# codex-storage/codex-storage-proofs-circuits

Measured on AMD Instinct MI355X. Metric: Poseidon2-BN254 permutations/sec per GPU; full proof-input witnesses/sec, higher is better.
Workload: dtype u32x9 (29-bit limbs, Montgomery mod BN254 r)

## Files before the change

### codex-storage-proofs-circuits_amd/csrc/proof_many.cpp

```cpp
#include <hip/hip_runtime.h>

#include <algorithm>
#include <cstring>
#include <map>
#include <memory>
#include <string>
#include <vector>

#include "dataset_obj.hpp"
#include "proof_input_obj.hpp"
#include "trees.hpp"

using namespace cp2i;

namespace {

struct Req {
  cp2_dataset* ds = nullptr;
  uint64_t slot = 0;
  uint8_t entropy[32];
  size_t at = 0;
  size_t id = 0;
};

// ... 14 lines not shown
    const cp2_dataset* d = ds[i];
    if (!d) return refuse(ctx, i, "NULL dataset");
    if (d->ctx != ctx) return refuse(ctx, i, "its dataset belongs to another context");
    const cp2_config& c = d->cfg;
    if (!same_circuit(c, ds[0]->cfg))
      return refuse(ctx, i, "its circuit parameters (maxDepth, maxLog2NSlots, cellSize, blockSize, nSamples) differ from request 0's");
    const uint64_t s = slot_idx[i];
    if (s < d->first_slot || s - d->first_slot >= d->n_local)
      return refuse(ctx, i, "slot " + std::to_string(s) + " is not local to its dataset (slots " + std::to_string(d->first_slot) + " .. " +
                                std::to_string(d->first_slot + d->n_local - 1) + ")");
    if (!d->have_roots && !(d->first_slot == 0 && d->n_local == c.n_slots))
      return refuse(ctx, i, "its dataset has no dataset tree: not all of its slots are local and cp2_dataset_set_roots was never called");
    const std::string shape = proof_shape_refusal(c, config_slot_tree_depth(c), config_dataset_tree_depth(c));
    if (!shape.empty()) return refuse(ctx, i, shape);
    if (!d->trees && d->tree_mode == 2 && d->csizes.size() - 1 != depth_of(c.n_cells / (c.block_size / c.cell_size)))
      return refuse(ctx, i, "its compact layers do not match its configuration");
  }
  return CP2_OK;
}

int check_roots(cp2_ctx* ctx, cp2_dataset* const* ds, const uint64_t* slot_idx, size_t n) {
  std::vector<uint64_t> a(n);
  for (size_t i = 0; i < n; ++i)
    a[i] = (uint64_t)reinterpret_cast<uintptr_t>(dataset_roots_dev(ds[i])) + (slot_idx[i] - ds[i]->first_slot) * 32;
  std::vector<uint8_t> got(n * 32);
  DevBuf d_a, d_r;
  CP2_TRY(d_a.scratch(ctx, n * 8));
  CP2_TRY(d_r.scratch(ctx, n * 32));
  CP2_HIP(ctx, hipMemcpyAsync(d_a.p, a.data(), n * 8, hipMemcpyHostToDevice, ctx->stream));
  CP2_HIP(ctx, cp2k::launch_gather_addr(static_cast<const uint64_t*>(d_a.p), n, 32, d_r.p, ctx->stream));
  CP2_HIP(ctx, hipMemcpyAsync(got.data(), d_r.p, n * 32, hipMemcpyDeviceToHost, ctx->stream));
  CP2_HIP(ctx, hipStreamSynchronize(ctx->stream));
  for (size_t i = 0; i < n; ++i)
    if (std::memcmp(&got[i * 32], &ds[i]->dlayers[slot_idx[i] * 32], 32) != 0)
      return refuse(ctx, i, "the root its dataset tree holds for slot " + std::to_string(slot_idx[i]) +
                                " (cp2_dataset_set_roots) differs from the slot's built root");
  return CP2_OK;
}

int prepare(cp2_ctx* ctx, cp2_dataset* const* ds, const uint64_t* slot_idx, size_t n) {
  CP2_TRY(validate(ctx, ds, slot_idx, n));
  CP2_HIP(ctx, hipSetDevice(ctx->device));
  std::vector<cp2_dataset*> bare;
  for (size_t i = 0; i < n; ++i)
    if (!ds[i]->have_roots) bare.push_back(ds[i]);
  std::sort(bare.begin(), bare.end());
  bare.erase(std::unique(bare.begin(), bare.end()), bare.end());
  CP2_TRY(set_roots_pass(ctx, bare.data(), nullptr, bare.size(), nullptr));
  return check_roots(ctx, ds, slot_idx, n);
}

std::string who(bool named, const Req* r) { return named ? "request " + std::to_string(r->id) + ": " : std::string(); }

int run_pass(cp2_ctx* ctx, const std::vector<const Req*>& rq, size_t n_rf, size_t n_rfile, size_t n_cf, bool named, cp2_proof_input** out) {
  const size_t n = rq.size(), nr = n_rf + n_rfile;
  const cp2_config& c0 = rq[0]->ds->cfg;
  const size_t ns = c0.n_samples, md = (size_t)c0.max_depth, cs = c0.cell_size, bs = c0.block_size, cpb = bs / cs;
  const size_t T = n * ns, R = nr * ns, C = T - R, RF = n_rf * ns, CF = n_cf * ns;
  auto store = std::make_shared<BatchStore>();
  if (T) {
    std::vector<cp2k::ManyReq> reqs(n);
    std::vector<cp2k::TreeGeom> geoms;
    std::map<std::string, uint32_t> geom_of;
    for (size_t j = 0; j < n; ++j) {
      const cp2_dataset* ds = rq[j]->ds;
      cp2k::ManyReq& q = reqs[j];
      std::memset(&q, 0, sizeof q);
      std::memcpy(q.entropy, rq[j]->entropy, 32);
      std::memcpy(q.slot_root, &ds->dlayers[rq[j]->slot * 32], 32);
      q.n_cells = ds->cfg.n_cells;
      q.cpb = cpb;
      if (j < nr) {
        cp2k::TreeGeom g;
        std::memset(&g, 0, sizeof g);
        trees_geom(ds->trees, &g);
        auto it = geom_of.emplace(std::string(reinterpret_cast<const char*>(&g), sizeof g), (uint32_t)geoms.size());
        if (it.second) geoms.push_back(g);
        q.geom = it.first->second;
        q.nodes = (uint64_t)reinterpret_cast<uintptr_t>(ds->trees->nodes.p);
        q.slot = rq[j]->slot - ds->first_slot;
      }
    }
    std::vector<uint64_t> blk(C), gen, cpaths, ctail, ccell;
    std::vector<uint8_t> checks(2 * C * 32);
    PinBuf h_blocks;
    const size_t rows = T * md + T + 2 * C;
    DevBuf d_req, d_geom, d_idx, d_blk, d_addr, d_rows, d_cells, d_gen, d_caddr;
    CP2_TRY(d_req.scratch(ctx, n * sizeof(cp2k::ManyReq)));
    CP2_TRY(d_geom.scratch(ctx, std::max<size_t>(1, geoms.size()) * sizeof(cp2k::TreeGeom)));
    CP2_TRY(d_idx.scratch(ctx, T * 8));
    CP2_TRY(d_blk.scratch(ctx, T * 8));
    CP2_TRY(d_addr.scratch(ctx, rows * 8));
    CP2_TRY(d_rows.scratch(ctx, rows * 32));
    CP2_TRY(d_cells.scratch(ctx, (C * cpb + T) * cs));
    CP2_TRY(store->idx.alloc(ctx, T * 8));
    CP2_TRY(store->paths.alloc(ctx, T * md * 32));
    CP2_TRY(store->leaves.alloc(ctx, T * 32));
    CP2_TRY(store->cells.alloc(ctx, T * cs));
    uint8_t* cells_out = d_cells.u8() + C * cpb * cs;
    uint64_t* addr = static_cast<uint64_t*>(d_addr.p);
    CP2_HIP(ctx, hipMemcpyAsync(d_req.p, reqs.data(), n * sizeof(cp2k::ManyReq), hipMemcpyHostToDevice, ctx->stream));
    if (!geoms.empty())
      CP2_HIP(ctx, hipMemcpyAsync(d_geom.p, geoms.data(), geoms.size() * sizeof(cp2k::TreeGeom), hipMemcpyHostToDevice, ctx->stream));
    CP2_HIP(ctx, cp2k::launch_sample_many(static_cast<const cp2k::ManyReq*>(d_req.p), static_cast<const cp2k::TreeGeom*>(d_geom.p), n,
                                          (uint32_t)ns, (uint32_t)md, static_cast<uint64_t*>(d_idx.p), static_cast<uint64_t*>(d_blk.p), addr,
                                          ctx->stream));
    CP2_HIP(ctx, hipMemcpyAsync(store->idx.p, d_idx.p, T * 8, hipMemcpyDeviceToHost, ctx->stream));
    if (C) CP2_HIP(ctx, hipMemcpyAsync(blk.data(), static_cast<uint64_t*>(d_blk.p) + R, C * 8, hipMemcpyDeviceToHost, ctx->stream));
    CP2_HIP(ctx, hipStreamSynchronize(ctx->stream));
    const uint64_t* idx = static_cast<const uint64_t*>(store->idx.p);

    gen.assign((CF + RF) * 2, 0);
    uint64_t* seeds = gen.data();
    uint64_t* firsts = seeds + CF + RF;
    for (size_t q = 0; q < CF; ++q) {
      const Req* r = rq[nr + q / ns];
      seeds[q] = cp2_slot_seed(r->ds->cfg.seed, r->slot);
      firsts[q] = blk[q] * cpb;
    }
    for (size_t p = 0; p < RF; ++p) {
      const Req* r = rq[p / ns];
      seeds[CF + p] = cp2_slot_seed(r->ds->cfg.seed, r->slot);
      firsts[CF + p] = idx[p];
    }
    if (CF + RF) {
      CP2_TRY(d_gen.scratch(ctx, gen.size() * 8));
      const uint64_t* dg = static_cast<const uint64_t*>(d_gen.p);
      CP2_HIP(ctx, hipMemcpyAsync(d_gen.p, gen.data(), gen.size() * 8, hipMemcpyHostToDevice, ctx->stream));
      CP2_HIP(ctx, cp2k::launch_gen_fake_cells_many(dg, dg + CF + RF, cpb, CF * cpb, cs, d_cells.p, ctx->stream));
      CP2_HIP(ctx, cp2k::launch_gen_fake_cells_many(dg + CF, dg + CF + RF + CF, 1, RF, cs, cells_out, ctx->stream));
    }
    if (C > CF) {
      const size_t n_req_file = (C - CF) / ns;
      CP2_TRY(h_blocks.alloc(ctx, (C - CF) * bs));
      std::vector<std::string> failed(fill_threads(ctx));
      on_threads(fill_threads(ctx), n_req_file, [&](int w, size_t k) {
        const size_t q0 = CF + k * ns;
        const Req* r = rq[nr + q0 / ns];
        const std::string fname = slot_file_name(r->ds->file_base, r->slot);
        size_t bad = 0;
        const int err = slot_file_read_list(fname, ns, [&](size_t) { return bs; }, [&](size_t c) { return blk[q0 + c] * bs; },
                                            [&](size_t c) { return h_blocks.u8() + (q0 - CF + c) * bs; }, &bad);
        if (err >= 0)
          failed[w] = who(named, r) + (err ? "block " + std::to_string(blk[q0 + bad]) + " of slot " : std::string("slot ")) + std::to_string(r->slot) +
                      ": " + slot_file_error(fname, err);
        return err < 0;
      });
      for (const auto& f : failed)
        if (!f.empty()) { ctx->err = f; return CP2_ERR_IO; }
      CP2_HIP(ctx, hipMemcpyAsync(d_cells.u8() + CF * bs, h_blocks.p, (C - CF) * bs, hipMemcpyHostToDevice, ctx->stream));
    }
    cp2_slot_trees* mini = nullptr;
    struct Mini { cp2_slot_trees*& t; ~Mini() { cp2_slot_trees_free(t); } } mini_guard{mini};
    if (C) {
      cpaths.assign(C * md, 0);
      ctail.assign(3 * C, 0);
      ccell.assign(C, 0);
      CP2_TRY(cp2_slot_trees_build_dev(ctx, d_cells.p, C, cs, bs, cpb, &mini));
      const size_t depth_b = depth_of(cpb);
      const uint64_t mb = (uint64_t)reinterpret_cast<uintptr_t>(mini->nodes.p);
      std::vector<uint64_t> rr(depth_b + 1);
      for (size_t q = 0; q < C; ++q) {
        const Req* r = rq[nr + q / ns];
        const cp2_dataset* ds = r->ds;
        const uint64_t ls = r->slot - ds->first_slot, cell = idx[R + q], b = blk[q], in_block = cell % cpb;
        const uint64_t kb = (uint64_t)reinterpret_cast<uintptr_t>(ds->compact.p);
        uint64_t* P = &cpaths[q * md];
        path_rows(mini, q, in_block, depth_b + 1, rr.data());
        for (size_t d = 0; d < depth_b; ++d) P[d] = rr[d] == NO_ROW ? 0 : mb + rr[d] * 32;
        uint64_t j = b, m = ds->cfg.n_cells / cpb;
        for (size_t d = 0; d + 1 < ds->csizes.size(); ++d) {
          const uint64_t sib = j ^ 1;
          P[depth_b + d] = sib < m ? kb + (ds->coff[d] + ls * ds->csizes[d] + sib) * 32 : 0;
          j >>= 1;
          m = (m + 1) >> 1;
        }
        ctail[q] = mb + (q * cpb + in_block) * 32;
        ctail[C + 2 * q] = kb + (ds->coff[0] + ls * ds->csizes[0] + b) * 32;
        ctail[C + 2 * q + 1] = mb + (mini->toff[0] + q) * 32;
        ccell[q] = (uint64_t)reinterpret_cast<uintptr_t>(d_cells.u8()) + (q * cpb + in_block) * cs;
      }
      CP2_TRY(d_caddr.scratch(ctx, C * 8));
      CP2_HIP(ctx, hipMemcpyAsync(addr + R * md, cpaths.data(), C * md * 8, hipMemcpyHostToDevice, ctx->stream));
      CP2_HIP(ctx, hipMemcpyAsync(addr + T * md + R, ctail.data(), 3 * C * 8, hipMemcpyHostToDevice, ctx->stream));
      CP2_HIP(ctx, hipMemcpyAsync(d_caddr.p, ccell.data(), C * 8, hipMemcpyHostToDevice, ctx->stream));
      CP2_HIP(ctx, cp2k::launch_gather_addr(static_cast<const uint64_t*>(d_caddr.p), C, cs, cells_out + R * cs, ctx->stream));
    }
    CP2_HIP(ctx, cp2k::launch_gather_addr(addr, rows, 32, d_rows.p, ctx->stream));
    CP2_HIP(ctx, hipMemcpyAsync(store->paths.p, d_rows.p, T * md * 32, hipMemcpyDeviceToHost, ctx->stream));
    CP2_HIP(ctx, hipMemcpyAsync(store->leaves.p, d_rows.u8() + T * md * 32, T * 32, hipMemcpyDeviceToHost, ctx->stream));
    if (C) CP2_HIP(ctx, hipMemcpyAsync(checks.data(), d_rows.u8() + (T * md + T) * 32, 2 * C * 32, hipMemcpyDeviceToHost, ctx->stream));
    CP2_HIP(ctx, hipMemcpyAsync(store->cells.p, cells_out, T * cs, hipMemcpyDeviceToHost, ctx->stream));
    CP2_HIP(ctx, hipStreamSynchronize(ctx->stream));
    for (size_t q = 0; q < C; ++q)
      if (std::memcmp(&checks[2 * q * 32], &checks[(2 * q + 1) * 32], 32) != 0) {
        const Req* r = rq[nr + q / ns];
        ctx->err = who(named, r) + "block " + std::to_string(blk[q]) + " of slot " + std::to_string(r->slot) +
                   " does not hash to its stored root (slot data changed since the build?)";
        return CP2_ERR_IO;
      }
    if (R > RF) {
      std::vector<std::string> failed(fill_threads(ctx));
      on_threads(fill_threads(ctx), n_rfile, [&](int w, size_t k) {
        const Req* r = rq[n_rf + k];
        const std::string fname = slot_file_name(r->ds->file_base, r->slot);
        const size_t p0 = (n_rf + k) * ns;
        const int err = slot_file_read_list(fname, ns, [&](size_t) { return cs; }, [&](size_t c) { return idx[p0 + c] * cs; },
                                            [&](size_t c) { return store->cells.u8() + (p0 + c) * cs; });
        if (err >= 0) failed[w] = who(named, r) + slot_file_error(fname, err);
        return err < 0;
      });
      for (const auto& f : failed)
        if (!f.empty()) { ctx->err = f; return CP2_ERR_IO; }
    }
  }
  std::vector<ProofItem> items(n);
  for (size_t j = 0; j < n; ++j) items[j] = {rq[j]->ds, rq[j]->slot, rq[j]->entropy, &out[rq[j]->at]};
  return proof_inputs_from_store(items.data(), n, store, store->cells.u8());
}

}

int cp2i::prove_requests(cp2_ctx* ctx, cp2_dataset* const* ds, const uint64_t* slot_idx, const uint8_t* entropies, size_t n, size_t at0,
                         bool named, cp2_proof_input** out) {
  for (size_t i = 0; i < n; ++i) out[i] = nullptr;
  if (n == 0) return CP2_OK;
  CP2_HIP(ctx, hipSetDevice(ctx->device));
  std::vector<Req> req(n);
  std::vector<const Req*> res_fake, res_file, cmp_fake, cmp_file, roots_only;
  for (size_t i = 0; i < n; ++i) {
    req[i].ds = ds[i];
    req[i].slot = slot_idx[i];
    req[i].at = i;
    req[i].id = at0 + i;
    canonical_felt(entropies + 32 * i, req[i].entropy);
    const cp2_dataset* d = ds[i];
    (d->trees ? (d->from_file ? res_file : res_fake) : d->tree_mode == 2 ? (d->from_file ? cmp_file : cmp_fake) : roots_only).push_back(&req[i]);
  }
  auto fail = [&](int st) {
    for (size_t i = 0; i < n; ++i) { cp2_proof_input_free(out[i]); out[i] = nullptr; }
    return st;
  };
  for (const Req* r : roots_only) {
    const int st = cp2_proof_inputs_generate_batch(r->ds, &r->slot, 1, r->entropy, &out[r->at]);
    if (st != CP2_OK) {
      ctx->err = who(named, r) + ctx->err;
      return fail(st);
    }
  }
  const cp2_config& c0 = ds[0]->cfg;
  const size_t per_req = std::max<size_t>(1, (size_t)c0.n_samples * c0.block_size);
  const size_t chunk = std::max<size_t>(1, ctx->stage_bytes / per_req);
  std::vector<const Req*> compact(cmp_fake);
  compact.insert(compact.end(), cmp_file.begin(), cmp_file.end());
  const size_t n_res = res_fake.size() + res_file.size();
  size_t c = 0;
  for (bool first = true; first ? n_res + compact.size() > 0 : c < compact.size(); first = false) {
    std::vector<const Req*> rq;
    if (first) {
      rq = res_fake;
      rq.insert(rq.end(), res_file.begin(), res_file.end());
    }
    const size_t c1 = std::min(compact.size(), c + chunk);
    rq.insert(rq.end(), compact.begin() + (long)c, compact.begin() + (long)c1);
    const size_t n_cf = c < cmp_fake.size() ? std::min(c1, cmp_fake.size()) - c : 0;
    const int st = run_pass(ctx, rq, first ? res_fake.size() : 0, first ? res_file.size() : 0, n_cf, named, out);
    if (st != CP2_OK) return fail(st);
    c = c1;
  }
  return CP2_OK;
}

extern "C" int cp2_proof_inputs_generate_many(cp2_ctx* ctx, cp2_dataset* const* ds, const uint64_t* slot_idx, const uint8_t* entropies, size_t n,
                                              cp2_proof_input** out) try {
  if (!ctx) return CP2_ERR_INVALID;
  if (n && (!ds || !slot_idx || !entropies || !out)) {
    ctx->err = "cp2_proof_inputs_generate_many: NULL array";
    return CP2_ERR_INVALID;
  }
  for (size_t i = 0; i < n; ++i) out[i] = nullptr;
  if (n == 0) return CP2_OK;
  CP2_REFUSE_STUCK(ctx);
  CP2_TRY(prepare(ctx, ds, slot_idx, n));
  return prove_requests(ctx, ds, slot_idx, entropies, n, 0, true, out);
} catch (const std::bad_alloc&) {
  return CP2_ERR_ALLOC;
} catch (...) {
  return CP2_ERR_INVALID;
}

extern "C" int cp2_proof_inputs_export_many(cp2_ctx* ctx, cp2_dataset* const* ds, const uint64_t* slot_idx, const uint8_t* entropies, size_t n,
                                            const char* const* paths, int threads, size_t batch, uint64_t* total_bytes) try {
  if (!ctx) return CP2_ERR_INVALID;
  if (n && (!ds || !slot_idx || !entropies)) {
    ctx->err = "cp2_proof_inputs_export_many: NULL array";
    return CP2_ERR_INVALID;
  }
  if (total_bytes) *total_bytes = 0;
  if (n == 0) return CP2_OK;
  CP2_REFUSE_STUCK(ctx);
  CP2_TRY(prepare(ctx, ds, slot_idx, n));
  return export_in_chunks(n, batch, threads, [&](size_t b0, size_t m, cp2_proof_input** out) {
    return prove_requests(ctx, ds + b0, slot_idx + b0, entropies + 32 * b0, m, b0, true, out);
  }, [&](size_t i) { return paths ? paths[i] : nullptr; }, total_bytes);
} catch (const std::bad_alloc&) {
  return CP2_ERR_ALLOC;
} catch (...) {
  return CP2_ERR_INVALID;
}
```

### codex-storage-proofs-circuits_amd/csrc/slot_trees.cpp

```cpp
#include <hip/hip_runtime.h>

#include <fcntl.h>
#include <sys/mman.h>
#include <sys/stat.h>
#include <unistd.h>

#include <algorithm>
#include <atomic>
#include <chrono>
#include <cstdio>
#include <cstdlib>
#include <cstring>
#include <memory>
#include <new>
#include <string>
#include <vector>

#include "trees.hpp"
#include "fake_turns.hpp"
#include "ingest_turns.hpp"
#include "fill_pipeline.hpp"

using namespace cp2i;

// ... 240 lines not shown
    st = sched.hashed_on(s);
    if (st == CP2_OK) st = sched.advance(c0 + n, c0 + n == total_cells, s);
  }
  if (scratch) scratch->tail_stream = sched.layer_stream();
  int fin = sched.finish();
  trace.lap("fake slots: generate + hash + layers");
  if (st == CP2_OK) st = fin;
  if (st != CP2_OK) return st;
  *out = t.release();
  return CP2_OK;
}

extern "C" int cp2_slot_trees_build_fake(cp2_ctx* ctx, uint64_t dataset_seed, uint64_t first_slot, size_t n_slots,
                                         size_t cell_size, size_t block_size, size_t n_cells, cp2_slot_trees** out) try {
  if (!ctx || !out) return CP2_ERR_INVALID;
  return trees_build_fake(ctx, dataset_seed, first_slot, n_slots, cell_size, block_size, n_cells, 0, nullptr, out);
} catch (const std::bad_alloc&) {
  return CP2_ERR_ALLOC;
} catch (...) {
  return CP2_ERR_INVALID;
}

bool cp2i::unit_geometry_ok(uint64_t units_per_slot, size_t cell_size, size_t block_size, size_t cells_per_unit) {
  if (!is_pow2(units_per_slot) || cell_size == 0 || block_size < cell_size) return false;
  const size_t nb = cells_per_unit / (block_size / cell_size);
  return nb >= 2 && is_pow2(nb);
}
extern "C" int cp2_slot_trees_build_fake_units(cp2_ctx* ctx, uint64_t dataset_seed, uint64_t units_per_slot, uint64_t first_unit,
                                               size_t n_units, size_t cell_size, size_t block_size, size_t cells_per_unit,
                                               cp2_slot_trees** out) try {
  if (!ctx || !out || units_per_slot == 0) return CP2_ERR_INVALID;
  CP2_TRY(trees_check_geometry(cell_size, block_size, cells_per_unit, n_units));
  if (units_per_slot > 1 && !unit_geometry_ok(units_per_slot, cell_size, block_size, cells_per_unit)) return CP2_ERR_INVALID;
  return trees_build_fake(ctx, dataset_seed, first_unit, n_units, cell_size, block_size, cells_per_unit, 0, nullptr, out, units_per_slot);
} catch (const std::bad_alloc&) {
  return CP2_ERR_ALLOC;
} catch (...) {
  return CP2_ERR_INVALID;
}

extern "C" int cp2_slot_trees_build_file_units(cp2_ctx* ctx, const char* file_base, uint64_t units_per_slot, uint64_t first_unit,
                                               size_t n_units, size_t cell_size, size_t block_size, size_t cells_per_unit,
                                               cp2_slot_trees** out) try {
  if (!ctx || !out || !file_base || units_per_slot == 0 || cell_size > SLOT_FILE_MAX_CELL) return CP2_ERR_INVALID;
  CP2_TRY(trees_check_geometry(cell_size, block_size, cells_per_unit, n_units));
  if (units_per_slot > 1 && !unit_geometry_ok(units_per_slot, cell_size, block_size, cells_per_unit)) return CP2_ERR_INVALID;
  return trees_build_files(ctx, file_base, first_unit, n_units, cell_size, block_size, cells_per_unit, 0, nullptr, out, units_per_slot);
} catch (const std::bad_alloc&) {
  return CP2_ERR_ALLOC;
} catch (...) {
  return CP2_ERR_INVALID;
}

extern "C" int cp2_slot_trees_build_dev(cp2_ctx* ctx, const void* d_cells, size_t n_slots, size_t cell_size,
                                        size_t block_size, size_t n_cells, cp2_slot_trees** out) try {
  if (!ctx || !out || !d_cells) return CP2_ERR_INVALID;
  *out = nullptr;
  CP2_REFUSE_STUCK(ctx);
  CP2_TRY(trees_check_geometry(cell_size, block_size, n_cells, n_slots));
  CP2_HIP(ctx, hipSetDevice(ctx->device));
  std::unique_ptr<cp2_slot_trees> t(trees_new(ctx, n_slots, cell_size, block_size, n_cells));
  if (!t) return CP2_ERR_ALLOC;
  t->src = CellSrc::Dev;
  t->d_cells = static_cast<const uint8_t*>(d_cells);
  CP2_TRY(trees_layout(t.get()));
  CP2_HIP(ctx, cp2k::launch_hash_cells(d_cells, cell_size, n_slots * n_cells, t->nodes.p, ctx->stream));
  CP2_TRY(trees_build_layers(t.get(), 0, n_slots, ctx->stream));
  *out = t.release();
  return CP2_OK;
} catch (const std::bad_alloc&) {
  return CP2_ERR_ALLOC;
} catch (...) {
  return CP2_ERR_INVALID;
}

namespace {

size_t env_size(const char* name, size_t dflt) {
  const char* v = std::getenv(name);
  if (!v || !*v) return dflt;
  char* end = nullptr;
  unsigned long long x = std::strtoull(v, &end, 10);
  return (end && *end == 0 && x > 0) ? (size_t)x : dflt;
}

struct IngestPipe {
  static constexpr int MAX_DEPTH = 8;
  static constexpr size_t DIRECT_ALIGN = 4096;
  size_t cell_multiple = 1;
  cp2_ctx* ctx = nullptr;
  hipStream_t copy = nullptr;
  int pin_depth = 0, dev_depth = 0;
  PinBuf pinned[MAX_DEPTH];
  DevBuf dev[MAX_DEPTH];
  hipEvent_t copied[MAX_DEPTH] = {};
  hipEvent_t uploaded[MAX_DEPTH] = {};
  hipEvent_t hashed[MAX_DEPTH] = {};
  size_t chunk = 0;
  size_t cap_bytes = 0;
  size_t turn = 0;
  size_t pin_turn = 0;
  int threads = 1;
  bool serial = false;
  hipStream_t hash_stream[2] = {nullptr, nullptr};
  int last_aux_dev = -1;

  ~IngestPipe() {
    if (!ctx) return;
    fill_join_all();
    const bool trace = std::getenv("CP2_TRACE") != nullptr && (mapped_chunks + ring_chunks) > 0;
    const double t0 = now_ms();
    (void)hipSetDevice(ctx->device);
    (void)finish();
    (void)hipStreamSynchronize(ctx->stream);
    if (hash_stream[1]) (void)hipStreamSynchronize(hash_stream[1]);
    if (copy) (void)hipStreamSynchronize(copy);
    const double t1 = now_ms();
    for (auto& mp : mappings) mp.open = false;
    (void)release_mapped();
    const double t2 = now_ms();
// ... 590 lines not shown
```

### codex-storage-proofs-circuits_amd/csrc/trees.hpp

```cpp
#pragma once
#include <functional>
#include <string>
#include <vector>

#include "batch_loop.hpp"
#include "internal.hpp"
#include "kernels.hpp"
#include "fill_pipeline.hpp"
#include "cache_file.hpp"

struct cp2_slot_trees {
  cp2_ctx* ctx = nullptr;
  size_t n_slots = 0, cell_size = 0, block_size = 0, n_cells = 0, cpb = 0, nblocks = 0;
  std::vector<size_t> bsizes, tsizes;
  std::vector<size_t> boff, toff;
  cp2i::DevBuf nodes;
  CellSrc src = CellSrc::Fake;
  uint64_t dataset_seed = 0, first_slot = 0;
  uint64_t units_per_slot = 1;
  bool pooled_nodes = false;
  const uint8_t* d_cells = nullptr;
  const uint8_t* h_cells = nullptr;
  std::string file_base;
};
// ... 21 lines not shown
                     size_t n_cells, size_t group, const SlotsDone& done, cp2_slot_trees** out, uint64_t units_per_slot = 1,
                     bool pooled_nodes = false, BuildScratch* scratch = nullptr, int node_slot = 0);
int trees_build_files(cp2_ctx* ctx, const std::string& base, uint64_t first_slot, size_t n_slots, size_t cell_size,
                      size_t block_size, size_t n_cells, size_t group, const SlotsDone& done, cp2_slot_trees** out,
                      uint64_t units_per_slot = 1, bool pooled_nodes = false, BuildScratch* scratch = nullptr, int node_slot = 0);
int trees_build_file_list(cp2_ctx* ctx, const std::string* names, size_t n_names, size_t cell_size, size_t block_size, size_t n_cells,
                          size_t group, const SlotsDone& done, cp2_slot_trees** out, bool pooled_nodes = false,
                          BuildScratch* scratch = nullptr, int node_slot = 0);
struct ItemSource {
  bool from_file = false;
  std::string file_base;
  uint64_t seed = 0;
  size_t cell_size = 0, block_size = 0, n_cells = 0;
  uint64_t units_per_slot = 1;
  const std::string* names = nullptr;
  size_t n_names = 0;
};
ItemSource item_source_of(const cp2_slot_trees* t, uint64_t units_per_slot);
ItemSource item_source_of(const cp2_dataset* ds);
int build_items(cp2_ctx* ctx, const ItemSource& src, uint64_t s0, size_t n, size_t group, const SlotsDone& done, cp2_slot_trees** out,
                bool pooled_nodes = false, BuildScratch* scratch = nullptr, int node_slot = 0);

struct BatchDevice {
  using Tail = hipStream_t;
  cp2_ctx* ctx = nullptr;
  BuildScratch scratch;
  Event landed[2];
  cp2_slot_trees* batch = nullptr;
  ~BatchDevice() { release(); }
  int init(cp2_ctx* c) { ctx = c; CP2_TRY(landed[0].create(c)); return landed[1].create(c); }
  int wait(int b) { return cleared(hipEventSynchronize(landed[b]) == hipSuccess); }
  int record(int b, hipStream_t tail) {
    if (hipEventRecord(landed[b], tail) == hipSuccess) return CP2_OK;
    ctx->err = "hipEventRecord failed";
    return CP2_ERR_HIP;
  }
  int drain() {
    return cleared(hipStreamSynchronize(ctx->stream) == hipSuccess && (!ctx->aux_stream || hipStreamSynchronize(ctx->aux_stream) == hipSuccess) &&
                   (!ctx->aux2_stream || hipStreamSynchronize(ctx->aux2_stream) == hipSuccess));
  }
  void release() { cp2_slot_trees_free(batch); batch = nullptr; }
  int build(const ItemSource& src, uint64_t s0, size_t n, size_t group, const SlotsDone& done, int b, hipStream_t* tail) {
    const int st = build_items(ctx, src, s0, n, group, done, &batch, true, &scratch, b);
    *tail = scratch.tail_stream ? scratch.tail_stream : ctx->stream;
    return st;
  }
  static int cleared(bool ok) { if (!ok) (void)hipGetLastError(); return ok ? CP2_OK : CP2_ERR_HIP; }
};

size_t trees_node_bytes(size_t n_slots, size_t cell_size, size_t block_size, size_t n_cells);
inline size_t trees_batch_items(const cp2_ctx* ctx, size_t cell_size, size_t block_size, size_t n_cells, uint64_t n_items) {
  return batch_items(ctx->stage_bytes, trees_node_bytes(1, cell_size, block_size, n_cells), n_items);
}
void trees_geom(const cp2_slot_trees* t, cp2k::TreeGeom* g);
void path_rows(const cp2_slot_trees* t, size_t slot, uint64_t cell, size_t max_depth, uint64_t* rows);
int trees_paths_multi(cp2_slot_trees* t, const uint64_t* slot_idx, const uint64_t* cell_idx, size_t n, size_t max_depth, uint8_t* out, uint8_t* leaf_hashes);
std::string slot_file_name(const std::string& base, uint64_t slot);
bool is_pow2(uint64_t x);

int kept_save(cp2_ctx* ctx, const char* path, CacheHead meta, const void* d_buf, size_t bytes);
int kept_load(cp2_ctx* ctx, const char* path, const CacheHead& want, void* d_buf, size_t bytes);

int dataset_own_roots_in_place(cp2_dataset* ds, bool* ok);

int scrub_items(cp2_ctx* ctx, const ItemSource& src, uint64_t item0, uint64_t n, int level, const uint8_t* kept, size_t kstride, size_t cap,
                std::vector<uint64_t>& bad, uint64_t* n_bad);
int dataset_scrub_level(const cp2_dataset* ds);
int dataset_scrub(cp2_dataset* ds, uint64_t first_slot, uint64_t n, int level, size_t cap, std::vector<uint64_t>& bad, uint64_t* n_bad);

bool stream_serial();

struct StageTimer {
  bool on;
  double t0;
  StageTimer();
  void lap(const char* what);
};

}
```

Baseline: 726.7 million.

## Double-buffer proof-input passes and sample all requests in one launch

Sampling now runs once up front for every request instead of once per pass. Passes are double-buffered across two PassSets, so host planning and file reads for the next chunk can overlap the GPU work still in flight for the previous one. Per-pass device and pinned buffers are grown and reused rather than reallocated, and the mini-tree layout and path tables are planned on the host before hashing is enqueued. This adds memory pressure, which is handled by falling back to a single set when allocation fails, and it makes error handling and lifetimes more complex.

Measured after the change: 726.8 million, median of 6. About the same (+0.0%).

```diff
diff --git a/codex-storage-proofs-circuits_amd/csrc/proof_many.cpp b/codex-storage-proofs-circuits_amd/csrc/proof_many.cpp
--- a/codex-storage-proofs-circuits_amd/csrc/proof_many.cpp
+++ b/codex-storage-proofs-circuits_amd/csrc/proof_many.cpp
@@ -90,172 +90,300 @@
 
 std::string who(bool named, const Req* r) { return named ? "request " + std::to_string(r->id) + ": " : std::string(); }
 
-int run_pass(cp2_ctx* ctx, const std::vector<const Req*>& rq, size_t n_rf, size_t n_rfile, size_t n_cf, bool named, cp2_proof_input** out) {
-  const size_t n = rq.size(), nr = n_rf + n_rfile;
-  const cp2_config& c0 = rq[0]->ds->cfg;
-  const size_t ns = c0.n_samples, md = (size_t)c0.max_depth, cs = c0.cell_size, bs = c0.block_size, cpb = bs / cs;
-  const size_t T = n * ns, R = nr * ns, C = T - R, RF = n_rf * ns, CF = n_cf * ns;
-  auto store = std::make_shared<BatchStore>();
-  if (T) {
-    std::vector<cp2k::ManyReq> reqs(n);
-    std::vector<cp2k::TreeGeom> geoms;
-    std::map<std::string, uint32_t> geom_of;
-    for (size_t j = 0; j < n; ++j) {
-      const cp2_dataset* ds = rq[j]->ds;
-      cp2k::ManyReq& q = reqs[j];
-      std::memset(&q, 0, sizeof q);
-      std::memcpy(q.entropy, rq[j]->entropy, 32);
-      std::memcpy(q.slot_root, &ds->dlayers[rq[j]->slot * 32], 32);
-      q.n_cells = ds->cfg.n_cells;
-      q.cpb = cpb;
-      if (j < nr) {
-        cp2k::TreeGeom g;
-        std::memset(&g, 0, sizeof g);
-        trees_geom(ds->trees, &g);
-        auto it = geom_of.emplace(std::string(reinterpret_cast<const char*>(&g), sizeof g), (uint32_t)geoms.size());
-        if (it.second) geoms.push_back(g);
-        q.geom = it.first->second;
-        q.nodes = (uint64_t)reinterpret_cast<uintptr_t>(ds->trees->nodes.p);
-        q.slot = rq[j]->slot - ds->first_slot;
-      }
-    }
-    std::vector<uint64_t> blk(C), gen, cpaths, ctail, ccell;
-    std::vector<uint8_t> checks(2 * C * 32);
-    PinBuf h_blocks;
-    const size_t rows = T * md + T + 2 * C;
-    DevBuf d_req, d_geom, d_idx, d_blk, d_addr, d_rows, d_cells, d_gen, d_caddr;
-    CP2_TRY(d_req.scratch(ctx, n * sizeof(cp2k::ManyReq)));
-    CP2_TRY(d_geom.scratch(ctx, std::max<size_t>(1, geoms.size()) * sizeof(cp2k::TreeGeom)));
-    CP2_TRY(d_idx.scratch(ctx, T * 8));
-    CP2_TRY(d_blk.scratch(ctx, T * 8));
-    CP2_TRY(d_addr.scratch(ctx, rows * 8));
-    CP2_TRY(d_rows.scratch(ctx, rows * 32));
-    CP2_TRY(d_cells.scratch(ctx, (C * cpb + T) * cs));
-    CP2_TRY(store->idx.alloc(ctx, T * 8));
-    CP2_TRY(store->paths.alloc(ctx, T * md * 32));
-    CP2_TRY(store->leaves.alloc(ctx, T * 32));
-    CP2_TRY(store->cells.alloc(ctx, T * cs));
-    uint8_t* cells_out = d_cells.u8() + C * cpb * cs;
-    uint64_t* addr = static_cast<uint64_t*>(d_addr.p);
-    CP2_HIP(ctx, hipMemcpyAsync(d_req.p, reqs.data(), n * sizeof(cp2k::ManyReq), hipMemcpyHostToDevice, ctx->stream));
-    if (!geoms.empty())
-      CP2_HIP(ctx, hipMemcpyAsync(d_geom.p, geoms.data(), geoms.size() * sizeof(cp2k::TreeGeom), hipMemcpyHostToDevice, ctx->stream));
-    CP2_HIP(ctx, cp2k::launch_sample_many(static_cast<const cp2k::ManyReq*>(d_req.p), static_cast<const cp2k::TreeGeom*>(d_geom.p), n,
-                                          (uint32_t)ns, (uint32_t)md, static_cast<uint64_t*>(d_idx.p), static_cast<uint64_t*>(d_blk.p), addr,
-                                          ctx->stream));
-    CP2_HIP(ctx, hipMemcpyAsync(store->idx.p, d_idx.p, T * 8, hipMemcpyDeviceToHost, ctx->stream));
-    if (C) CP2_HIP(ctx, hipMemcpyAsync(blk.data(), static_cast<uint64_t*>(d_blk.p) + R, C * 8, hipMemcpyDeviceToHost, ctx->stream));
-    CP2_HIP(ctx, hipStreamSynchronize(ctx->stream));
-    const uint64_t* idx = static_cast<const uint64_t*>(store->idx.p);
-
-    gen.assign((CF + RF) * 2, 0);
-    uint64_t* seeds = gen.data();
-    uint64_t* firsts = seeds + CF + RF;
-    for (size_t q = 0; q < CF; ++q) {
-      const Req* r = rq[nr + q / ns];
+struct Call {
+  cp2_ctx* ctx = nullptr;
+  bool named = false;
+  cp2_proof_input** out = nullptr;
+  std::vector<const Req*> order;
+  size_t n_rf = 0, n_rfile = 0, n_cfake = 0;
+  size_t ns = 0, md = 0, cs = 0, bs = 0, cpb = 0;
+  std::vector<cp2k::ManyReq> reqs;
+  std::vector<cp2k::TreeGeom> geoms;
+  PinBuf h_sampled;
+  DevBuf d_req, d_geom, d_idx, d_blk, d_addr;
+  size_t nr() const { return n_rf + n_rfile; }
+  size_t lanes() const { return order.size() * ns; }
+  size_t R() const { return nr() * ns; }
+  const uint64_t* idx() const { return static_cast<const uint64_t*>(h_sampled.p); }
+  const uint64_t* blk() const { return idx() + lanes(); }
+};
+
+int sample(Call& k) {
+  cp2_ctx* ctx = k.ctx;
+  const size_t n = k.order.size(), nr = k.nr(), T = k.lanes(), R = k.R(), C = T - R;
+  if (!T) return CP2_OK;
+  k.reqs.resize(n);
+  std::map<std::string, uint32_t> geom_of;
+  for (size_t j = 0; j < n; ++j) {
+    const Req* r = k.order[j];
+    const cp2_dataset* ds = r->ds;
+    cp2k::ManyReq& q = k.reqs[j];
+    std::memset(&q, 0, sizeof q);
+    std::memcpy(q.entropy, r->entropy, 32);
+    std::memcpy(q.slot_root, &ds->dlayers[r->slot * 32], 32);
+    q.n_cells = ds->cfg.n_cells;
+    q.cpb = k.cpb;
+    if (j < nr) {
+      cp2k::TreeGeom g;
+      std::memset(&g, 0, sizeof g);
+      trees_geom(ds->trees, &g);
+      auto it = geom_of.emplace(std::string(reinterpret_cast<const char*>(&g), sizeof g), (uint32_t)k.geoms.size());
+      if (it.second) k.geoms.push_back(g);
+      q.geom = it.first->second;
+      q.nodes = (uint64_t)reinterpret_cast<uintptr_t>(ds->trees->nodes.p);
+      q.slot = r->slot - ds->first_slot;
+    }
+  }
+  CP2_TRY(k.h_sampled.alloc(ctx, (T + C) * 8));
+  CP2_TRY(k.d_req.scratch(ctx, n * sizeof(cp2k::ManyReq)));
+  CP2_TRY(k.d_geom.scratch(ctx, std::max<size_t>(1, k.geoms.size()) * sizeof(cp2k::TreeGeom)));
+  CP2_TRY(k.d_idx.scratch(ctx, T * 8));
+  CP2_TRY(k.d_blk.scratch(ctx, T * 8));
+  CP2_TRY(k.d_addr.scratch(ctx, R ? (T * k.md + R) * 8 : 0));
+  uint64_t* host = static_cast<uint64_t*>(k.h_sampled.p);
+  CP2_HIP(ctx, hipMemcpyAsync(k.d_req.p, k.reqs.data(), n * sizeof(cp2k::ManyReq), hipMemcpyHostToDevice, ctx->stream));
+  if (!k.geoms.empty())
+    CP2_HIP(ctx, hipMemcpyAsync(k.d_geom.p, k.geoms.data(), k.geoms.size() * sizeof(cp2k::TreeGeom), hipMemcpyHostToDevice, ctx->stream));
+  CP2_HIP(ctx, cp2k::launch_sample_many(static_cast<const cp2k::ManyReq*>(k.d_req.p), static_cast<const cp2k::TreeGeom*>(k.d_geom.p), n,
+                                        (uint32_t)k.ns, (uint32_t)k.md, static_cast<uint64_t*>(k.d_idx.p), static_cast<uint64_t*>(k.d_blk.p),
+                                        static_cast<uint64_t*>(k.d_addr.p), ctx->stream));
+  CP2_HIP(ctx, hipMemcpyAsync(host, k.d_idx.p, T * 8, hipMemcpyDeviceToHost, ctx->stream));
+  if (C) CP2_HIP(ctx, hipMemcpyAsync(host + T, static_cast<uint64_t*>(k.d_blk.p) + R, C * 8, hipMemcpyDeviceToHost, ctx->stream));
+  CP2_HIP(ctx, hipStreamSynchronize(ctx->stream));
+  return CP2_OK;
+}
+
+struct Pass {
+  size_t n_rf = 0, n_rfile = 0;
+  size_t c0 = 0, c1 = 0, n_cf = 0;
+};
+
+struct Dim {
+  size_t n, nr, T, R, C, RF, CF, G, rows;
+};
+Dim dims(const Call& k, const Pass& p) {
+  Dim d;
+  d.nr = p.n_rf + p.n_rfile;
+  d.n = d.nr + (p.c1 - p.c0);
+  d.T = d.n * k.ns;
+  d.R = d.nr * k.ns;
+  d.C = d.T - d.R;
+  d.RF = p.n_rf * k.ns;
+  d.CF = p.n_cf * k.ns;
+  d.G = d.CF + d.RF;
+  d.rows = d.T * k.md + d.T + 2 * d.C;
+  return d;
+}
+
+int grow(cp2_ctx* ctx, DevBuf& b, size_t n) { return b.p && b.bytes >= n ? CP2_OK : b.scratch(ctx, n); }
+int grow(cp2_ctx* ctx, PinBuf& b, size_t n) { return b.p && b.bytes >= n ? CP2_OK : b.alloc(ctx, n); }
+
+struct PassSet {
+  cp2_ctx* ctx = nullptr;
+  Pass pass;
+  bool in_flight = false;
+  PinBuf h_tab;
+  PinBuf h_blocks, h_checks;
+  std::shared_ptr<BatchStore> store;
+  DevBuf d_tab, d_addr, d_rows, d_cells, d_nodes;
+  cp2_slot_trees* mini = nullptr;
+  Event done;
+  PassSet() = default;
+  PassSet(const PassSet&) = delete;
+  PassSet& operator=(const PassSet&) = delete;
+  ~PassSet() {
+    drain();
+    cp2_slot_trees_free(mini);
+  }
+  void drain() {
+    if (in_flight && ctx && !ctx->stuck) {
+      (void)hipSetDevice(ctx->device);
+      if (hipStreamSynchronize(ctx->stream) != hipSuccess) (void)hipGetLastError();
+    }
+    in_flight = false;
+  }
+  void release() {
+    cp2_slot_trees_free(mini);
+    mini = nullptr;
+    store.reset();
+    d_tab.release(); d_addr.release(); d_rows.release(); d_cells.release(); d_nodes.release();
+    h_tab.release(); h_blocks.release(); h_checks.release();
+  }
+
+  const Req* request(const Call& k, size_t j) const {
+    const size_t nr = pass.n_rf + pass.n_rfile;
+    return j < nr ? k.order[j] : k.order[k.nr() + pass.c0 + (j - nr)];
+  }
+  const Req* compact_request(const Call& k, size_t q) const { return k.order[k.nr() + pass.c0 + q / k.ns]; }
+  const uint64_t* lane_idx(const Call& k) const { return k.idx() + k.R() + pass.c0 * k.ns - (pass.n_rf + pass.n_rfile) * k.ns; }
+  const uint64_t* lane_blk(const Call& k) const { return k.blk() + pass.c0 * k.ns; }
+
+  int reserve(const Call& k, const Pass& p) {
+    ctx = k.ctx;
+    pass = p;
+    const Dim d = dims(k, p);
+    cp2_slot_trees_free(mini);
+    mini = nullptr;
+    store = std::make_shared<BatchStore>();
+    if (!d.T) return CP2_OK;
+    if (!done.e) CP2_TRY(done.create(ctx));
+    CP2_TRY(grow(ctx, h_tab, (2 * d.G + d.C + d.C * k.md + 3 * d.C) * 8));
+    if (d.C > d.CF) CP2_TRY(grow(ctx, h_blocks, (d.C - d.CF) * k.bs));
+    if (d.C) CP2_TRY(grow(ctx, h_checks, 2 * d.C * 32));
+    CP2_TRY(grow(ctx, d_tab, (2 * d.G + d.C) * 8));
+    CP2_TRY(grow(ctx, d_addr, d.rows * 8));
+    CP2_TRY(grow(ctx, d_rows, d.rows * 32));
+    CP2_TRY(grow(ctx, d_cells, (d.C * k.cpb + d.T) * k.cs));
+    CP2_TRY(store->idx.alloc(ctx, d.T * 8));
+    CP2_TRY(store->paths.alloc(ctx, d.T * k.md * 32));
+    CP2_TRY(store->leaves.alloc(ctx, d.T * 32));
+    CP2_TRY(store->cells.alloc(ctx, d.T * k.cs));
+    if (d.C) {
+      if (trees_check_geometry(k.cs, k.bs, k.cpb, d.C) != CP2_OK) return CP2_ERR_INVALID;
+      mini = trees_new(ctx, d.C, k.cs, k.bs, k.cpb);
+      if (!mini) return CP2_ERR_ALLOC;
+      CP2_TRY(trees_layout(mini, &d_nodes));
+    }
+    return CP2_OK;
+  }
+
+  void plan(const Call& k) {
+    const Dim d = dims(k, pass);
+    if (!d.T) return;
+    const size_t ns = k.ns, md = k.md, cs = k.cs, cpb = k.cpb;
+    const uint64_t *idx = lane_idx(k), *blk = lane_blk(k);
+    std::memcpy(store->idx.p, idx, d.T * 8);
+    uint64_t* seeds = static_cast<uint64_t*>(h_tab.p);
+    uint64_t *firsts = seeds + d.G, *ccell = seeds + 2 * d.G, *cpaths = ccell + d.C, *ctail = cpaths + d.C * md;
+    for (size_t q = 0; q < d.CF; ++q) {
+      const Req* r = compact_request(k, q);
       seeds[q] = cp2_slot_seed(r->ds->cfg.seed, r->slot);
       firsts[q] = blk[q] * cpb;
     }
-    for (size_t p = 0; p < RF; ++p) {
-      const Req* r = rq[p / ns];
-      seeds[CF + p] = cp2_slot_seed(r->ds->cfg.seed, r->slot);
-      firsts[CF + p] = idx[p];
-    }
-    if (CF + RF) {
-      CP2_TRY(d_gen.scratch(ctx, gen.size() * 8));
-      const uint64_t* dg = static_cast<const uint64_t*>(d_gen.p);
-      CP2_HIP(ctx, hipMemcpyAsync(d_gen.p, gen.data(), gen.size() * 8, hipMemcpyHostToDevice, ctx->stream));
-      CP2_HIP(ctx, cp2k::launch_gen_fake_cells_many(dg, dg + CF + RF, cpb, CF * cpb, cs, d_cells.p, ctx->stream));
-      CP2_HIP(ctx, cp2k::launch_gen_fake_cells_many(dg + CF, dg + CF + RF + CF, 1, RF, cs, cells_out, ctx->stream));
-    }
-    if (C > CF) {
-      const size_t n_req_file = (C - CF) / ns;
-      CP2_TRY(h_blocks.alloc(ctx, (C - CF) * bs));
+    for (size_t t = 0; t < d.RF; ++t) {
+      const Req* r = k.order[t / ns];
+      seeds[d.CF + t] = cp2_slot_seed(r->ds->cfg.seed, r->slot);
+      firsts[d.CF + t] = idx[t];
+    }
+    if (!d.C) return;
+    std::memset(cpaths, 0, d.C * md * 8);
+    const size_t depth_b = depth_of(cpb);
+    const uint64_t mb = (uint64_t)reinterpret_cast<uintptr_t>(mini->nodes.p);
+    std::vector<uint64_t> rr(depth_b + 1);
+    for (size_t q = 0; q < d.C; ++q) {
+      const Req* r = compact_request(k, q);
+      const cp2_dataset* ds = r->ds;
+      const uint64_t ls = r->slot - ds->first_slot, cell = idx[d.R + q], b = blk[q], in_block = cell % cpb;
+      const uint64_t kb = (uint64_t)reinterpret_cast<uintptr_t>(ds->compact.p);
+      uint64_t* P = &cpaths[q * md];
+      path_rows(mini, q, in_block, depth_b + 1, rr.data());
+      for (size_t e = 0; e < depth_b; ++e) P[e] = rr[e] == NO_ROW ? 0 : mb + rr[e] * 32;
+      uint64_t j = b, m = ds->cfg.n_cells / cpb;
+      for (size_t e = 0; e + 1 < ds->csizes.size(); ++e) {
+        const uint64_t sib = j ^ 1;
+        P[depth_b + e] = sib < m ? kb + (ds->coff[e] + ls * ds->csizes[e] + sib) * 32 : 0;
+        j >>= 1;
+        m = (m + 1) >> 1;
+      }
+      ctail[q] = mb + (q * cpb + in_block) * 32;
+      ctail[d.C + 2 * q] = kb + (ds->coff[0] + ls * ds->csizes[0] + b) * 32;
+      ctail[d.C + 2 * q + 1] = mb + (mini->toff[0] + q) * 32;
+      ccell[q] = (uint64_t)reinterpret_cast<uintptr_t>(d_cells.u8()) + (q * cpb + in_block) * cs;
+    }
+  }
+
+  int enqueue(const Call& k) {
+    const Dim d = dims(k, pass);
+    if (!d.T) return CP2_OK;
+    const size_t ns = k.ns, md = k.md, cs = k.cs, bs = k.bs, cpb = k.cpb;
+    const uint64_t* tab = static_cast<const uint64_t*>(h_tab.p);
+    const uint64_t* blk = lane_blk(k);
+    uint64_t* addr = static_cast<uint64_t*>(d_addr.p);
+    uint8_t* cells_out = d_cells.u8() + d.C * cpb * cs;
+    const uint64_t* dg = static_cast<const uint64_t*>(d_tab.p);
+    in_flight = true;
+    if (2 * d.G + d.C) CP2_HIP(ctx, hipMemcpyAsync(d_tab.p, tab, (2 * d.G + d.C) * 8, hipMemcpyHostToDevice, ctx->stream));
+    if (d.G) {
+      CP2_HIP(ctx, cp2k::launch_gen_fake_cells_many(dg, dg + d.G, cpb, d.CF * cpb, cs, d_cells.p, ctx->stream));
+      CP2_HIP(ctx, cp2k::launch_gen_fake_cells_many(dg + d.CF, dg + d.G + d.CF, 1, d.RF, cs, cells_out, ctx->stream));
+    }
+    if (d.C > d.CF) {
+      const size_t n_req_file = (d.C - d.CF) / ns;
       std::vector<std::string> failed(fill_threads(ctx));
-      on_threads(fill_threads(ctx), n_req_file, [&](int w, size_t k) {
-        const size_t q0 = CF + k * ns;
-        const Req* r = rq[nr + q0 / ns];
+      on_threads(fill_threads(ctx), n_req_file, [&](int w, size_t f) {
+        const size_t q0 = d.CF + f * ns;
+        const Req* r = compact_request(k, q0);
         const std::string fname = slot_file_name(r->ds->file_base, r->slot);
         size_t bad = 0;
         const int err = slot_file_read_list(fname, ns, [&](size_t) { return bs; }, [&](size_t c) { return blk[q0 + c] * bs; },
-                                            [&](size_t c) { return h_blocks.u8() + (q0 - CF + c) * bs; }, &bad);
+                                            [&](size_t c) { return h_blocks.u8() + (q0 - d.CF + c) * bs; }, &bad);
         if (err >= 0)
-          failed[w] = who(named, r) + (err ? "block " + std::to_string(blk[q0 + bad]) + " of slot " : std::string("slot ")) + std::to_string(r->slot) +
-                      ": " + slot_file_error(fname, err);
+          failed[w] = who(k.named, r) + (err ? "block " + std::to_string(blk[q0 + bad]) + " of slot " : std::string("slot ")) +
+                      std::to_string(r->slot) + ": " + slot_file_error(fname, err);
         return err < 0;
       });
       for (const auto& f : failed)
         if (!f.empty()) { ctx->err = f; return CP2_ERR_IO; }
-      CP2_HIP(ctx, hipMemcpyAsync(d_cells.u8() + CF * bs, h_blocks.p, (C - CF) * bs, hipMemcpyHostToDevice, ctx->stream));
-    }
-    cp2_slot_trees* mini = nullptr;
-    struct Mini { cp2_slot_trees*& t; ~Mini() { cp2_slot_trees_free(t); } } mini_guard{mini};
-    if (C) {
-      cpaths.assign(C * md, 0);
-      ctail.assign(3 * C, 0);
-      ccell.assign(C, 0);
-      CP2_TRY(cp2_slot_trees_build_dev(ctx, d_cells.p, C, cs, bs, cpb, &mini));
-      const size_t depth_b = depth_of(cpb);
-      const uint64_t mb = (uint64_t)reinterpret_cast<uintptr_t>(mini->nodes.p);
-      std::vector<uint64_t> rr(depth_b + 1);
-      for (size_t q = 0; q < C; ++q) {
-        const Req* r = rq[nr + q / ns];
-        const cp2_dataset* ds = r->ds;
-        const uint64_t ls = r->slot - ds->first_slot, cell = idx[R + q], b = blk[q], in_block = cell % cpb;
-        const uint64_t kb = (uint64_t)reinterpret_cast<uintptr_t>(ds->compact.p);
-        uint64_t* P = &cpaths[q * md];
-        path_rows(mini, q, in_block, depth_b + 1, rr.data());
-        for (size_t d = 0; d < depth_b; ++d) P[d] = rr[d] == NO_ROW ? 0 : mb + rr[d] * 32;
-        uint64_t j = b, m = ds->cfg.n_cells / cpb;
-        for (size_t d = 0; d + 1 < ds->csizes.size(); ++d) {
-          const uint64_t sib = j ^ 1;
-          P[depth_b + d] = sib < m ? kb + (ds->coff[d] + ls * ds->csizes[d] + sib) * 32 : 0;
-          j >>= 1;
-          m = (m + 1) >> 1;
+      CP2_HIP(ctx, hipMemcpyAsync(d_cells.u8() + d.CF * bs, h_blocks.p, (d.C - d.CF) * bs, hipMemcpyHostToDevice, ctx->stream));
+    }
+    if (d.C) {
+      CP2_TRY(trees_hash_dev(mini, d_cells.p));
+      CP2_HIP(ctx, hipMemcpyAsync(addr + d.R * md, tab + 2 * d.G + d.C, d.C * md * 8, hipMemcpyHostToDevice, ctx->stream));
+      CP2_HIP(ctx, hipMemcpyAsync(addr + d.T * md + d.R, tab + 2 * d.G + d.C + d.C * md, 3 * d.C * 8, hipMemcpyHostToDevice, ctx->stream));
+      CP2_HIP(ctx, cp2k::launch_gather_addr(dg + 2 * d.G, d.C, cs, cells_out + d.R * cs, ctx->stream));
+    }
+    if (d.R) {
+      const uint64_t* sa = static_cast<const uint64_t*>(k.d_addr.p);
+      CP2_HIP(ctx, hipMemcpyAsync(addr, sa, d.R * md * 8, hipMemcpyDeviceToDevice, ctx->stream));
+      CP2_HIP(ctx, hipMemcpyAsync(addr + d.T * md, sa + k.lanes() * md, d.R * 8, hipMemcpyDeviceToDevice, ctx->stream));
+    }
+    CP2_HIP(ctx, cp2k::launch_gather_addr(addr, d.rows, 32, d_rows.p, ctx->stream));
+    CP2_HIP(ctx, hipMemcpyAsync(store->paths.p, d_rows.p, d.T * md * 32, hipMemcpyDeviceToHost, ctx->stream));
+    CP2_HIP(ctx, hipMemcpyAsync(store->leaves.p, d_rows.u8() + d.T * md * 32, d.T * 32, hipMemcpyDeviceToHost, ctx->stream));
+    if (d.C) CP2_HIP(ctx, hipMemcpyAsync(h_checks.p, d_rows.u8() + (d.T * md + d.T) * 32, 2 * d.C * 32, hipMemcpyDeviceToHost, ctx->stream));
+    CP2_HIP(ctx, hipMemcpyAsync(store->cells.p, cells_out, d.T * cs, hipMemcpyDeviceToHost, ctx->stream));
+    CP2_HIP(ctx, hipEventRecord(done, ctx->stream));
+    return CP2_OK;
+  }
+
+  int finish(const Call& k) {
+    const Dim d = dims(k, pass);
+    const size_t ns = k.ns, cs = k.cs;
+    if (d.T) {
+      CP2_HIP(ctx, hipEventSynchronize(done));
+      in_flight = false;
+      const uint64_t *idx = lane_idx(k), *blk = lane_blk(k);
+      const uint8_t* checks = h_checks.u8();
+      for (size_t q = 0; q < d.C; ++q)
+        if (std::memcmp(&checks[2 * q * 32], &checks[(2 * q + 1) * 32], 32) != 0) {
+          const Req* r = compact_request(k, q);
+          ctx->err = who(k.named, r) + "block " + std::to_string(blk[q]) + " of slot " + std::to_string(r->slot) +
+                     " does not hash to its stored root (slot data changed since the build?)";
+          return CP2_ERR_IO;
         }
-        ctail[q] = mb + (q * cpb + in_block) * 32;
-        ctail[C + 2 * q] = kb + (ds->coff[0] + ls * ds->csizes[0] + b) * 32;
-        ctail[C + 2 * q + 1] = mb + (mini->toff[0] + q) * 32;
-        ccell[q] = (uint64_t)reinterpret_cast<uintptr_t>(d_cells.u8()) + (q * cpb + in_block) * cs;
+      if (d.R > d.RF) {
+        std::vector<std::string> failed(fill_threads(ctx));
+        on_threads(fill_threads(ctx), pass.n_rfile, [&](int w, size_t f) {
+          const Req* r = k.order[pass.n_rf + f];
+          const std::string fname = slot_file_name(r->ds->file_base, r->slot);
+          const size_t p0 = (pass.n_rf + f) * ns;
+          const int err = slot_file_read_list(fname, ns, [&](size_t) { return cs; }, [&](size_t c) { return idx[p0 + c] * cs; },
+                                              [&](size_t c) { return store->cells.u8() + (p0 + c) * cs; });
+          if (err >= 0) failed[w] = who(k.named, r) + slot_file_error(fname, err);
+          return err < 0;
+        });
+        for (const auto& f : failed)
+          if (!f.empty()) { ctx->err = f; return CP2_ERR_IO; }
       }
-      CP2_TRY(d_caddr.scratch(ctx, C * 8));
-      CP2_HIP(ctx, hipMemcpyAsync(addr + R * md, cpaths.data(), C * md * 8, hipMemcpyHostToDevice, ctx->stream));
-      CP2_HIP(ctx, hipMemcpyAsync(addr + T * md + R, ctail.data(), 3 * C * 8, hipMemcpyHostToDevice, ctx->stream));
-      CP2_HIP(ctx, hipMemcpyAsync(d_caddr.p, ccell.data(), C * 8, hipMemcpyHostToDevice, ctx->stream));
-      CP2_HIP(ctx, cp2k::launch_gather_addr(static_cast<const uint64_t*>(d_caddr.p), C, cs, cells_out + R * cs, ctx->stream));
-    }
-    CP2_HIP(ctx, cp2k::launch_gather_addr(addr, rows, 32, d_rows.p, ctx->stream));
-    CP2_HIP(ctx, hipMemcpyAsync(store->paths.p, d_rows.p, T * md * 32, hipMemcpyDeviceToHost, ctx->stream));
-    CP2_HIP(ctx, hipMemcpyAsync(store->leaves.p, d_rows.u8() + T * md * 32, T * 32, hipMemcpyDeviceToHost, ctx->stream));
-    if (C) CP2_HIP(ctx, hipMemcpyAsync(checks.data(), d_rows.u8() + (T * md + T) * 32, 2 * C * 32, hipMemcpyDeviceToHost, ctx->stream));
-    CP2_HIP(ctx, hipMemcpyAsync(store->cells.p, cells_out, T * cs, hipMemcpyDeviceToHost, ctx->stream));
-    CP2_HIP(ctx, hipStreamSynchronize(ctx->stream));
-    for (size_t q = 0; q < C; ++q)
-      if (std::memcmp(&checks[2 * q * 32], &checks[(2 * q + 1) * 32], 32) != 0) {
-        const Req* r = rq[nr + q / ns];
-        ctx->err = who(named, r) + "block " + std::to_string(blk[q]) + " of slot " + std::to_string(r->slot) +
-                   " does not hash to its stored root (slot data changed since the build?)";
-        return CP2_ERR_IO;
-      }
-    if (R > RF) {
-      std::vector<std::string> failed(fill_threads(ctx));
-      on_threads(fill_threads(ctx), n_rfile, [&](int w, size_t k) {
-        const Req* r = rq[n_rf + k];
-        const std::string fname = slot_file_name(r->ds->file_base, r->slot);
-        const size_t p0 = (n_rf + k) * ns;
-        const int err = slot_file_read_list(fname, ns, [&](size_t) { return cs; }, [&](size_t c) { return idx[p0 + c] * cs; },
-                                            [&](size_t c) { return store->cells.u8() + (p0 + c) * cs; });
-        if (err >= 0) failed[w] = who(named, r) + slot_file_error(fname, err);
-        return err < 0;
-      });
-      for (const auto& f : failed)
-        if (!f.empty()) { ctx->err = f; return CP2_ERR_IO; }
-    }
-  }
-  std::vector<ProofItem> items(n);
-  for (size_t j = 0; j < n; ++j) items[j] = {rq[j]->ds, rq[j]->slot, rq[j]->entropy, &out[rq[j]->at]};
-  return proof_inputs_from_store(items.data(), n, store, store->cells.u8());
-}
+    }
+    std::vector<ProofItem> items(d.n);
+    for (size_t j = 0; j < d.n; ++j) {
+      const Req* r = request(k, j);
+      items[j] = {r->ds, r->slot, r->entropy, &k.out[r->at]};
+    }
+    return proof_inputs_from_store(items.data(), d.n, store, store->cells.u8());
+  }
+};
 
 }
 
@@ -287,27 +415,75 @@
     }
   }
   const cp2_config& c0 = ds[0]->cfg;
-  const size_t per_req = std::max<size_t>(1, (size_t)c0.n_samples * c0.block_size);
+  Call k;
+  k.ctx = ctx;
+  k.named = named;
+  k.out = out;
+  k.ns = c0.n_samples;
+  k.md = (size_t)c0.max_depth;
+  k.cs = c0.cell_size;
+  k.bs = c0.block_size;
+  k.cpb = k.bs / k.cs;
+  k.n_rf = res_fake.size();
+  k.n_rfile = res_file.size();
+  k.n_cfake = cmp_fake.size();
+  for (const auto* v : {&res_fake, &res_file, &cmp_fake, &cmp_file}) k.order.insert(k.order.end(), v->begin(), v->end());
+  if (k.order.empty()) return CP2_OK;
+  const size_t n_compact = cmp_fake.size() + cmp_file.size();
+  const size_t per_req = std::max<size_t>(1, k.ns * k.bs);
   const size_t chunk = std::max<size_t>(1, ctx->stage_bytes / per_req);
-  std::vector<const Req*> compact(cmp_fake);
-  compact.insert(compact.end(), cmp_file.begin(), cmp_file.end());
-  const size_t n_res = res_fake.size() + res_file.size();
+  {
+    const int st = sample(k);
+    if (st != CP2_OK) return fail(st);
+  }
+  PassSet sets[2];
+  int flying = -1, only = -1;
   size_t c = 0;
-  for (bool first = true; first ? n_res + compact.size() > 0 : c < compact.size(); first = false) {
-    std::vector<const Req*> rq;
-    if (first) {
-      rq = res_fake;
-      rq.insert(rq.end(), res_file.begin(), res_file.end());
-    }
-    const size_t c1 = std::min(compact.size(), c + chunk);
-    rq.insert(rq.end(), compact.begin() + (long)c, compact.begin() + (long)c1);
-    const size_t n_cf = c < cmp_fake.size() ? std::min(c1, cmp_fake.size()) - c : 0;
-    const int st = run_pass(ctx, rq, first ? res_fake.size() : 0, first ? res_file.size() : 0, n_cf, named, out);
+  for (size_t pi = 0; pi == 0 || c < n_compact; ++pi) {
+    Pass p;
+    if (pi == 0) { p.n_rf = k.n_rf; p.n_rfile = k.n_rfile; }
+    p.c0 = c;
+    p.c1 = std::min(n_compact, c + chunk);
+    p.n_cf = c < k.n_cfake ? std::min(p.c1, k.n_cfake) - c : 0;
+    c = p.c1;
+    int s = only >= 0 ? only : (int)(pi & 1);
+    if (flying == s) {
+      const int st = sets[s].finish(k);
+      flying = -1;
+      if (st != CP2_OK) return fail(st);
+    }
+    int st = sets[s].reserve(k, p);
+    if (st == CP2_ERR_ALLOC && flying >= 0) {
+      sets[s].release();
+      only = s = flying;
+      flying = -1;
+      st = sets[s].finish(k);
+      if (st != CP2_OK) return fail(st);
+      st = sets[s].reserve(k, p);
+    }
+    if (st == CP2_OK) {
+      sets[s].plan(k);
+      st = sets[s].enqueue(k);
+    }
+    const std::string err = st != CP2_OK ? ctx->err : std::string();
+    if (flying >= 0) {
+      const int before = sets[flying].finish(k);
+      flying = -1;
+      if (before != CP2_OK) return fail(before);
+    }
+    if (st != CP2_OK) {
+      ctx->err = err;
+      return fail(st);
+    }
+    flying = s;
+  }
+  if (flying >= 0) {
+    const int st = sets[flying].finish(k);
     if (st != CP2_OK) return fail(st);
-    c = c1;
   }
   return CP2_OK;
 }
+
 
 extern "C" int cp2_proof_inputs_generate_many(cp2_ctx* ctx, cp2_dataset* const* ds, const uint64_t* slot_idx, const uint8_t* entropies, size_t n,
                                               cp2_proof_input** out) try {
diff --git a/codex-storage-proofs-circuits_amd/csrc/slot_trees.cpp b/codex-storage-proofs-circuits_amd/csrc/slot_trees.cpp
--- a/codex-storage-proofs-circuits_amd/csrc/slot_trees.cpp
+++ b/codex-storage-proofs-circuits_amd/csrc/slot_trees.cpp
@@ -316,6 +316,14 @@
   return CP2_ERR_INVALID;
 }
 
+int cp2i::trees_hash_dev(cp2_slot_trees* t, const void* d_cells) {
+  cp2_ctx* ctx = t->ctx;
+  t->src = CellSrc::Dev;
+  t->d_cells = static_cast<const uint8_t*>(d_cells);
+  CP2_HIP(ctx, cp2k::launch_hash_cells(d_cells, t->cell_size, t->n_slots * t->n_cells, t->nodes.p, ctx->stream));
+  return trees_build_layers(t, 0, t->n_slots, ctx->stream);
+}
+
 extern "C" int cp2_slot_trees_build_dev(cp2_ctx* ctx, const void* d_cells, size_t n_slots, size_t cell_size,
                                         size_t block_size, size_t n_cells, cp2_slot_trees** out) try {
   if (!ctx || !out || !d_cells) return CP2_ERR_INVALID;
@@ -325,11 +333,8 @@
   CP2_HIP(ctx, hipSetDevice(ctx->device));
   std::unique_ptr<cp2_slot_trees> t(trees_new(ctx, n_slots, cell_size, block_size, n_cells));
   if (!t) return CP2_ERR_ALLOC;
-  t->src = CellSrc::Dev;
-  t->d_cells = static_cast<const uint8_t*>(d_cells);
   CP2_TRY(trees_layout(t.get()));
-  CP2_HIP(ctx, cp2k::launch_hash_cells(d_cells, cell_size, n_slots * n_cells, t->nodes.p, ctx->stream));
-  CP2_TRY(trees_build_layers(t.get(), 0, n_slots, ctx->stream));
+  CP2_TRY(trees_hash_dev(t.get(), d_cells));
   *out = t.release();
   return CP2_OK;
 } catch (const std::bad_alloc&) {
diff --git a/codex-storage-proofs-circuits_amd/csrc/trees.hpp b/codex-storage-proofs-circuits_amd/csrc/trees.hpp
--- a/codex-storage-proofs-circuits_amd/csrc/trees.hpp
+++ b/codex-storage-proofs-circuits_amd/csrc/trees.hpp
@@ -97,6 +97,7 @@
 inline size_t trees_batch_items(const cp2_ctx* ctx, size_t cell_size, size_t block_size, size_t n_cells, uint64_t n_items) {
   return batch_items(ctx->stage_bytes, trees_node_bytes(1, cell_size, block_size, n_cells), n_items);
 }
+int trees_hash_dev(cp2_slot_trees* t, const void* d_cells);
 void trees_geom(const cp2_slot_trees* t, cp2k::TreeGeom* g);
 void path_rows(const cp2_slot_trees* t, size_t slot, uint64_t cell, size_t max_depth, uint64_t* rows);
 int trees_paths_multi(cp2_slot_trees* t, const uint64_t* slot_idx, const uint64_t* cell_idx, size_t n, size_t max_depth, uint8_t* out, uint8_t* leaf_hashes);
```
